# Tencent/hpc-ops

Hardware: AMD Instinct MI355X
Metric: attention_decode_fp8_kv_throughput (higher is better)
Workload: dtype fp8_e4m3

## Files before the change

### hpc-ops_amd/csrc/attention_decode_v2.h

```cpp
#pragma once
#include <hip/hip_runtime.h>
#include <stdint.h>

#include "attention_decode_route.h"

namespace hpc {
namespace decode2 {

struct Args {
  const void* q;
  const void* kcache;
  const void* vcache;
  const int* block_ids;
  const int* lens;
  const int* task_map;
  uint16_t* y;
  float* part_o;
  float* part_lse;
  int* arrive;
  const float* qscale;
  const float* kscale;
  const float* vscale;
  int num_batch, num_seq_q, num_head_kv, g_shift, page_shift, max_blocks;
  int ldq, ldy, qscale_stride, new_kv_included;
  int share_shift = 0;
  int min_range_cost;
  int bf16;
  int ktok = 0;
  int pair_wgs[4];
  int big_pct;
  int dev_nomem;
  int pair_xor;
  int mate_from;
  int xcd_map;
  int dev_sleep;
  int dev_merge_dup = 0;
  int dev_nosnap = 0;
  int dev_slice;
  long k_block_stride, k_token_stride;
  long v_block_stride, v_token_stride;
  long ks_block_stride, ks_row_stride, ks_head_stride;
  int hnd = 0;
  long k_head_stride = 0, v_head_stride = 0;
  float scale_log2;
  void* prof;
};

int launch(Args a, const DecodeRoute& r, hipStream_t stream);
#ifdef HPC_DEV
int ticket_overruns(bool reset);
#endif

}
}
```

### hpc-ops_amd/csrc/attention_decode_v2.hip

```cpp
#include <atomic>
#include <type_traits>
#include <utility>

#include "hpc_common.h"
#include "hpc_dev.h"
#include "../../include/hpc_amd.h"
#include "attention_decode_v2.h"

namespace hpc {
namespace decode2 {

#ifdef HPC_DEV
__device__ int g_ticket_overruns;
#endif
constexpr int kThreads = 256;
constexpr int kWaves = 4;
constexpr float kNegInf = -__builtin_inff();
constexpr int kRow = 256;
constexpr int kRows = 32;
constexpr int kVOff = kRows * kRow;
constexpr int kWaveLds = 2 * kRows * kRow;

template <int kAux>
__device__ __forceinline__ void ld_x4x4(u32x4 (&k)[4], int voff, i32x4 rs_in, int s1, int s2, int s3) {
  const i32x4 rs = pin(rs_in);
  if constexpr (kAux == 2)
    asm volatile("s_nop 4\n\tbuffer_load_dwordx4 %0, %4, %5, 0 offen nt\n\tbuffer_load_dwordx4 %1, %4, %5, %6 offen nt\n\t"
                 "buffer_load_dwordx4 %2, %4, %5, %7 offen nt\n\tbuffer_load_dwordx4 %3, %4, %5, %8 offen nt"
                 : "=&v"(k[0]), "=&v"(k[1]), "=&v"(k[2]), "=&v"(k[3])
                 : "v"(voff), "s"(rs), "s"(s1), "s"(s2), "s"(s3));
  else
    asm volatile("s_nop 4\n\tbuffer_load_dwordx4 %0, %4, %5, 0 offen\n\tbuffer_load_dwordx4 %1, %4, %5, %6 offen\n\t"
                 "buffer_load_dwordx4 %2, %4, %5, %7 offen\n\tbuffer_load_dwordx4 %3, %4, %5, %8 offen"
                 : "=&v"(k[0]), "=&v"(k[1]), "=&v"(k[2]), "=&v"(k[3])
                 : "v"(voff), "s"(rs), "s"(s1), "s"(s2), "s"(s3));
}
__device__ __forceinline__ void ld_q3(u32x4 (&q)[2], uint32_t& sc, int voff_q, i32x4 rq_in, int voff_s, i32x4 rsc_in) {
  const i32x4 rq = pin(rq_in), rsc = pin(rsc_in);
  asm volatile("s_nop 4\n\tbuffer_load_dwordx4 %0, %3, %4, 0 offen\n\tbuffer_load_dwordx4 %1, %3, %4, 0 offen offset:64\n\t"
               "buffer_load_dword %2, %5, %6, 0 offen"
               : "=&v"(q[0]), "=&v"(q[1]), "=&v"(sc)
               : "v"(voff_q), "s"(rq), "v"(voff_s), "s"(rsc));
}
__device__ __forceinline__ void ld_q4(u32x4 (&q)[4], int voff_q, i32x4 rq_in) {
  const i32x4 rq = pin(rq_in);
  asm volatile("s_nop 4\n\tbuffer_load_dwordx4 %0, %4, %5, 0 offen\n\tbuffer_load_dwordx4 %1, %4, %5, 0 offen offset:64\n\t"
               "buffer_load_dwordx4 %2, %4, %5, 0 offen offset:128\n\tbuffer_load_dwordx4 %3, %4, %5, 0 offen offset:192"
               : "=&v"(q[0]), "=&v"(q[1]), "=&v"(q[2]), "=&v"(q[3])
               : "v"(voff_q), "s"(rq));
}
__device__ __forceinline__ void ld_ks(uint32_t& sc, int voff, i32x4 rs_in) {
  const i32x4 rs = pin(rs_in);
  asm volatile("s_nop 4\n\tbuffer_load_dword %0, %1, %2, 0 offen" : "=&v"(sc) : "v"(voff), "s"(rs));
}
template <int N>
__device__ __forceinline__ void wait_ks(uint32_t& sc) {
  asm volatile("s_waitcnt vmcnt(%1)" : "+v"(sc) : "n"(N));
}
template <int N>
__device__ __forceinline__ void wait_ks2(uint32_t& sc0, uint32_t& sc1) {
  asm volatile("s_waitcnt vmcnt(%2)" : "+v"(sc0), "+v"(sc1) : "n"(N));
}
template <int N>
__device__ __forceinline__ void wait_q8(u32x4 (&q0)[4], u32x4 (&q1)[4]) {
  asm volatile("s_waitcnt vmcnt(%8)"
               : "+v"(q0[0]), "+v"(q0[1]), "+v"(q0[2]), "+v"(q0[3]), "+v"(q1[0]), "+v"(q1[1]), "+v"(q1[2]), "+v"(q1[3])
               : "n"(N < 63 ? N : 63));
}
template <int N>
__device__ __forceinline__ void wait_x4x4(u32x4 (&k)[4]) {
  asm volatile("s_waitcnt vmcnt(%4)" : "+v"(k[0]), "+v"(k[1]), "+v"(k[2]), "+v"(k[3]) : "n"(N < 63 ? N : 63));
}
template <int N>
__device__ __forceinline__ void wait_q(u32x4 (&q0)[2], u32x4 (&q1)[2], uint32_t& s0, uint32_t& s1) {
  asm volatile("s_waitcnt vmcnt(%6)" : "+v"(q0[0]), "+v"(q0[1]), "+v"(q1[0]), "+v"(q1[1]), "+v"(s0), "+v"(s1) : "n"(N < 63 ? N : 63));
}


constexpr int kFValid = 1;
constexpr int kFLast = 2;
constexpr int kFFirst = 4;
constexpr int kFOn0 = 8;
constexpr int kFOn1 = 16;
constexpr int kFMasked = 32;

template <int kAux, bool kBf16 = false, bool kProf = false, bool kQuad = false, bool kKtok = false, bool kHnd = false, bool kSolo = false>
__global__ __launch_bounds__(kThreads, 2) void decode2_kernel(const Args a) {
  static_assert(!kSolo || (!kQuad && !kHnd), "one head per workgroup: fp8 (both quant types) or bf16");
  static_assert(!(kSolo && kBf16 && kKtok), "bf16 has no scales");
  static_assert(!(kBf16 && kQuad), "the quad form is fp8");
  static_assert(!kKtok || (!kBf16 && !kQuad), "per-token K scales: the fp8 head-pair form");
  static_assert(!kHnd || (!kBf16 && !kQuad && !kKtok), "HND pages: the fp8 head-pair form with per-tensor scales");
  __shared__ float s_ks[kKtok ? kWaves : 1][64];
  constexpr bool kWide = (kBf16 && !kSolo) || kQuad;
  constexpr bool kBSolo = kBf16 && kSolo;
  __shared__ __attribute__((aligned(1024))) uint8_t s_wave[kWaves][kWaveLds];
  __shared__ float s_m[2][kWaves][16];
  __shared__ float s_l[2][kWaves][16];
  __shared__ int s_ticket[2];
  constexpr int kH = kSolo ? 1 : kQuad ? 4 : 2;
  constexpr int kW = kBSolo ? 32 : kSolo ? 64 : kWide ? 16 : 32;
  constexpr int kRowB = kBSolo ? 256 : kSolo ? 128 : kWide ? 512 : 256;
  constexpr int kRpi = kBSolo ? 4 : (kHnd || kSolo) ? 8 : kWide ? 2 : 4;
  constexpr int kCpr = 64 / kRpi;

  const int tid = threadIdx.x;
  const int lane = tid & 63;
  const int wave = sgpr(tid >> 6);
  const int n = lane & 15;
  const int g = lane >> 4;
  const int wg = blockIdx.x, nwg = gridDim.x;
  const int B = a.num_batch, Sq = a.num_seq_q;
  const int G = 1 << a.g_shift;
  const int rows_valid = Sq << a.g_shift;
  auto row_ok = [&](int r16, int hh = 0) __attribute__((always_inline)) { return (kQuad ? (r16 & 7) : kSolo ? 16 * hh + r16 : r16) < rows_valid; };
  const int page_mask = (1 << a.page_shift) - 1;
  const cint_ptr lens = as_const(a.lens);
  const int mpl_tiles = as_const(a.task_map)[6] >> 6;
  const int add_new = a.new_kv_included ? 0 : Sq;
  const uint8_t* qbase = static_cast<const uint8_t*>(a.q);
  const auto part_rs = make_rsrc(a.part_o);
  const auto lse_rs = make_rsrc(a.part_lse);
  auto ltot_of = [&](int b) __attribute__((always_inline)) { const int l = lens[b] + add_new; return l > 0 ? l : 0; };
  auto tiles_of = [&](int b) __attribute__((always_inline)) { return (ltot_of(b) + 63) >> 6; };

  constexpr int kOvh = 2;
  auto cost_of = [&](int b) __attribute__((always_inline)) { const int t = tiles_of(b); return t > 0 ? t + kOvh : 0; };
  const int kpl = (B + 63) >> 6;
  int chunk_sum = 0;
  for (int i = 0; i < kpl; ++i) {
    const int b = lane * kpl + i;
    if (b < B) {
      const int l = a.lens[b] + add_new;
      const int t = ((l > 0 ? l : 0) + 63) >> 6;
      chunk_sum += t > 0 ? t + kOvh : 0;
    }
  }
  int incl = chunk_sum;
  incl += __builtin_amdgcn_update_dpp(0, incl, 0x111, 0xF, 0xF, false);
  incl += __builtin_amdgcn_update_dpp(0, incl, 0x112, 0xF, 0xF, false);
  incl += __builtin_amdgcn_update_dpp(0, incl, 0x114, 0xF, 0xF, false);
  incl += __builtin_amdgcn_update_dpp(0, incl, 0x118, 0xF, 0xF, false);
  incl += __builtin_amdgcn_update_dpp(0, incl, 0x142, 0xA, 0xF, false);
  incl += __builtin_amdgcn_update_dpp(0, incl, 0x143, 0xC, 0xF, false);
  const int chunk_start = incl - chunk_sum;
  const int Th = __builtin_amdgcn_readlane(incl, 63);
  const int npair = a.num_head_kv / kH;
  if (Th == 0) return;
  int nrange = nwg / npair;
  int rng = wg / npair;
  int pr = wg % npair;
  if (a.xcd_map != 0 && npair == 4 && (nwg & 7) == 0) {
    const int e = (a.xcd_map >> (3 * (wg & 7))) & 7;
    pr = e & 3;
    rng = (wg >> 3) * 2 + (e >> 2);
  }
  if (a.mate_from > 0 && wg >= a.mate_from) pr ^= a.pair_xor;
  if constexpr (kSolo) {
    if (a.share_shift > 0) {
      const int ss = a.share_shift, hk = npair >> ss;
// ... 3 lines not shown
        rng = (j >> ss) * (8 / hk) + x / hk;
      } else {
        pr = ((pr % hk) << ss) | (pr / hk);
      }
    }
  }
  int lwg = wg;
  int lwg0 = pr * nrange;
  if (a.pair_wgs[0] > 0 && npair == 4) {
    const int n0 = a.pair_wgs[0], n1 = a.pair_wgs[1], n2 = a.pair_wgs[2], n3 = a.pair_wgs[3];
    const int nmin = min(min(n0, n1), min(n2, n3));
    if (wg >= nmin * 4) {
      int e = wg - nmin * 4;
      pr = 0;
      rng = nmin + e;
      if (e >= n0 - nmin) { e -= n0 - nmin; pr = 1; rng = nmin + e;
        if (e >= n1 - nmin) { e -= n1 - nmin; pr = 2; rng = nmin + e;
          if (e >= n2 - nmin) { e -= n2 - nmin; pr = 3; rng = nmin + e; } } }
    }
    nrange = pr == 0 ? n0 : pr == 1 ? n1 : pr == 2 ? n2 : n3;
    lwg0 = pr == 0 ? 0 : pr == 1 ? n0 : pr == 2 ? n0 + n1 : n0 + n1 + n2;
  }
  lwg = lwg0 + rng;
  const int nbig = a.big_pct > 100 ? (nwg / 2) / npair : 0;
  const long denom = static_cast<long>(nbig) * a.big_pct + static_cast<long>(nrange - nbig) * 100;
  const int per_s_even = static_cast<int>((static_cast<long>(Th) * 100 + denom - 1) / denom);
  const int per_floor = a.min_range_cost > mpl_tiles ? a.min_range_cost : mpl_tiles;
  const int per_s = per_s_even > per_floor ? per_s_even : per_floor;
  const int per_b = nbig > 0 ? (per_s * a.big_pct + 99) / 100 : per_s;
  const int big_span = nbig * per_b;
  auto range_of = [&](int pos) __attribute__((always_inline)) { return pos < big_span ? pos / per_b : nbig + (pos - big_span) / per_s; };
  const long g_begin = rng < nbig ? static_cast<long>(rng) * per_b : big_span + static_cast<long>(rng - nbig) * per_s;
  const int per = rng < nbig ? per_b : per_s;
  const long g_end = g_begin + per < Th ? g_begin + per : Th;
  if (g_begin >= g_end) return;

  constexpr int kSnap = 16;
  const bool snap = per_s_even <= per_floor && !(kHpcDevBuild && a.dev_nosnap);
  auto locate = [&](int x, int& b_out, int& rt_out, int& cc_out) __attribute__((always_inline)) {
    if (x >= Th) {
      b_out = B;
      rt_out = 0;
      cc_out = Th;
      return;
    }
    const uint64_t le = __ballot(chunk_start <= x);
    const int cl = 63 - __builtin_clzll(le);
    int pos = __builtin_amdgcn_readlane(chunk_start, cl);
    int b = cl * kpl;
    while (true) {
      const int t = cost_of(b);
      if (x < pos + t) break;
      pos += t;
      ++b;
    }
    if (snap && x > pos) {
      const int t = cost_of(b);
      if (t - kOvh <= kSnap) {
        if (2 * (x - pos) >= t) {
          pos += t;
          ++b;
          while (b < B && cost_of(b) == 0) ++b;
          if (b >= B) {
            b_out = B;
            rt_out = 0;
            cc_out = Th;
            return;
          }
        }
        b_out = b;
        rt_out = 0;
        cc_out = pos;
        return;
      }
    }
    b_out = b;
    rt_out = x - pos > kOvh ? x - pos - kOvh : 0;
    cc_out = pos;
  };
  int c_b, c_rt0, c_cc, e_b, e_rt, e_cc;
  locate(static_cast<int>(g_begin), c_b, c_rt0, c_cc);
  locate(static_cast<int>(g_end), e_b, e_rt, e_cc);
  if (c_b == e_b && c_rt0 >= e_rt) return;

  int q0_b = 0, q0_ltot = 0, q0_end = 0, q0_cc = 0;
  int q1_b = 0, q1_ltot = 0, q1_end = 0, q1_cc = 0;
  int q2_b = 0, q2_ltot = 0, q2_end = 0, q2_cc = 0;
  int qn = 0;
  int c_tok = 0, c_tok_end = 0, c_ltot = 0, c_tiles = 0, c_first = 1, c_valid = 1, c_pending = 0, c_last = 0;
  cint_ptr c_row = as_const(a.block_ids);
  auto open_task = [&]() __attribute__((always_inline)) {
    c_ltot = ltot_of(c_b);
    c_tiles = (c_ltot + 63) >> 6;
    const int end_t = c_b == e_b ? e_rt : c_tiles;
    c_tok_end = end_t * 64 < c_ltot ? end_t * 64 : c_ltot;
    c_tok = c_rt0 * 64 + wave * kW;
    c_first = 1;
    c_row = as_const(a.block_ids) + static_cast<long>(c_b) * a.max_blocks;
    const bool e0 = qn == 0, e1 = qn == 1, e2 = qn >= 2;
    q0_b = e0 ? c_b : q0_b, q0_ltot = e0 ? c_ltot : q0_ltot, q0_end = e0 ? c_tok_end : q0_end, q0_cc = e0 ? c_cc : q0_cc;
    q1_b = e1 ? c_b : q1_b, q1_ltot = e1 ? c_ltot : q1_ltot, q1_end = e1 ? c_tok_end : q1_end, q1_cc = e1 ? c_cc : q1_cc;
    q2_b = e2 ? c_b : q2_b, q2_ltot = e2 ? c_ltot : q2_ltot, q2_end = e2 ? c_tok_end : q2_end, q2_cc = e2 ? c_cc : q2_cc;
    ++qn;
  };
  auto next_task = [&]() __attribute__((always_inline)) {
    if (c_b == e_b) {
      c_valid = 0;
      return;
    }
    c_cc += c_tiles + kOvh;
    do {
      ++c_b;
    } while (c_b < e_b && tiles_of(c_b) == 0);
    if (c_b == e_b && e_rt == 0) {
      c_valid = 0;
      return;
    }
    c_rt0 = 0;
    open_task();
  };
  const bool blk1_same_page = (1 << a.page_shift) >= kW;
  auto step = [&](int& tok, int& fl, int& pid0, int& pid1) __attribute__((always_inline)) {
    if (c_pending && c_valid) {
      if (c_last) {
        next_task();
      } else {
        c_tok += kWaves * kW;
        c_first = 0;
      }
    }
    c_pending = 1;
    c_last = c_tok + kWaves * kW >= c_tok_end;
    const bool on0 = c_valid && c_tok < c_tok_end, on1 = c_valid && c_tok + kW / 2 < c_tok_end;
    const bool masked = c_tok + kW > c_ltot - Sq + 1 || c_tok + kW > c_tok_end;
    fl = (c_valid ? kFValid : 0) | (c_last ? kFLast : 0) | (c_first ? kFFirst : 0) | (on0 ? kFOn0 : 0) | (on1 ? kFOn1 : 0) |
         (masked ? kFMasked : 0);
    tok = c_tok;
    pid0 = on0 ? c_row[c_tok >> a.page_shift] : 0;
    pid1 = (!blk1_same_page && on1) ? c_row[(c_tok + kW / 2) >> a.page_shift] : 0;
  };

  u32x4 kr[2][4];
  u32x4 vr[2][4];
  uint32_t qsc[2];
  const uint32_t k_rs = static_cast<uint32_t>(a.k_token_stride), v_rs = static_cast<uint32_t>(a.v_token_stride);
  const int in0 = (wave * kW) & page_mask;
  const int in1 = blk1_same_page ? in0 + kW / 2 : ((wave * kW + kW / 2) & page_mask);
  const int lane_off = (lane % kCpr) * 16;
  const int k_voff0 = static_cast<int>((in0 + lane / kCpr) * k_rs) + lane_off, k_voff1 = static_cast<int>((in1 + lane / kCpr) * k_rs) + lane_off;
  const int v_voff0 = static_cast<int>((in0 + lane / kCpr) * v_rs) + lane_off, v_voff1 = static_cast<int>((in1 + lane / kCpr) * v_rs) + lane_off;
  const int ks1 = sgpr(kRpi * k_rs), ks2 = sgpr(kHnd ? static_cast<uint32_t>(a.k_head_stride) : 2 * kRpi * k_rs);
  const int ks3 = sgpr(kHnd ? static_cast<uint32_t>(a.k_head_stride) + kRpi * k_rs : 3 * kRpi * k_rs);
  const int vs1 = sgpr(kRpi * v_rs), vs2 = sgpr(kHnd ? static_cast<uint32_t>(a.v_head_stride) : 2 * kRpi * v_rs);
  const int vs3 = sgpr(kHnd ? static_cast<uint32_t>(a.v_head_stride) + kRpi * v_rs : 3 * kRpi * v_rs);
  const int mem_slice = kSolo ? (pr >> a.share_shift) : (a.dev_slice > 0 ? a.dev_slice - 1 : pr);
  const uint64_t kbase_h = reinterpret_cast<uint64_t>(a.kcache) + static_cast<uint64_t>(mem_slice) * (kSolo ? static_cast<uint64_t>(a.k_head_stride) : kHnd ? 2 * static_cast<uint64_t>(a.k_head_stride) : kRowB);
  const uint64_t vbase_h = reinterpret_cast<uint64_t>(a.vcache) + static_cast<uint64_t>(mem_slice) * (kSolo ? static_cast<uint64_t>(a.v_head_stride) : kHnd ? 2 * static_cast<uint64_t>(a.v_head_stride) : kRowB);
  const uint32_t kbs = static_cast<uint32_t>(a.k_block_stride), vbs = static_cast<uint32_t>(a.v_block_stride);
  const bool mem = a.dev_nomem == 0;
  i32x4 dk0, dk1, dv0, dv1;
  uint32_t ksr = 0;
  uint32_t ksr1 = 0;
  i32x4 dks = i32x4{0, 0, 0, kSrdWord3};
  i32x4 dks1 = i32x4{0, 0, 0, kSrdWord3};
  const uint64_t ksbase_h = reinterpret_cast<uint64_t>(a.kscale) + static_cast<uint64_t>(mem_slice) * (kSolo ? 1 : 2) * a.ks_head_stride +
                            static_cast<uint64_t>(in0 >> 5) * a.ks_row_stride;
  const uint64_t ksbase1_h = reinterpret_cast<uint64_t>(a.kscale) + static_cast<uint64_t>(mem_slice) * a.ks_head_stride +
                             static_cast<uint64_t>(blk1_same_page ? (in0 >> 5) + 1 : in1 >> 5) * a.ks_row_stride;
  const uint32_t ksbs = static_cast<uint32_t>(a.ks_block_stride);
  auto make_descs = [&](int fl, int pid0, int pid1) __attribute__((always_inline)) {
    const int nrec0 = (fl & kFOn0) && mem ? -1 : 0, nrec1 = (fl & kFOn1) && mem ? -1 : 0;
    const uint64_t ka = kbase_h + static_cast<uint64_t>(static_cast<uint32_t>(pid0)) * kbs;
    const uint64_t va = vbase_h + static_cast<uint64_t>(static_cast<uint32_t>(pid0)) * vbs;
    dk0 = srd(static_cast<uint32_t>(ka), static_cast<uint32_t>(ka >> 32), nrec0);
    dv0 = srd(static_cast<uint32_t>(va), static_cast<uint32_t>(va >> 32), nrec0);
    if (blk1_same_page) {
      dk1 = i32x4{dk0[0], dk0[1], sgpr(nrec1), kSrdWord3};
      dv1 = i32x4{dv0[0], dv0[1], sgpr(nrec1), kSrdWord3};
    } else {
      const uint64_t kb = kbase_h + static_cast<uint64_t>(static_cast<uint32_t>(pid1)) * kbs;
      const uint64_t vb = vbase_h + static_cast<uint64_t>(static_cast<uint32_t>(pid1)) * vbs;
      dk1 = srd(static_cast<uint32_t>(kb), static_cast<uint32_t>(kb >> 32), nrec1);
      dv1 = srd(static_cast<uint32_t>(vb), static_cast<uint32_t>(vb >> 32), nrec1);
    }
    if constexpr (kKtok) {
      const uint64_t sa = ksbase_h + static_cast<uint64_t>(static_cast<uint32_t>(pid0)) * ksbs;
      dks = srd(static_cast<uint32_t>(sa), static_cast<uint32_t>(sa >> 32), (fl & kFOn0) ? (kSolo ? 128 : 256) : 0);
      if constexpr (kSolo) {
        const uint64_t sb = ksbase1_h + static_cast<uint64_t>(static_cast<uint32_t>(blk1_same_page ? pid0 : pid1)) * ksbs;
        dks1 = srd(static_cast<uint32_t>(sb), static_cast<uint32_t>(sb >> 32), (fl & kFOn1) ? 128 : 0);
      }
    }
  };
  auto issue_k0 = [&]() __attribute__((always_inline)) { ld_x4x4<kAux>(kr[0], k_voff0, dk0, ks1, ks2, ks3); };
  auto issue_k1 = [&]() __attribute__((always_inline)) { ld_x4x4<kAux>(kr[1], k_voff1, dk1, ks1, ks2, ks3); };
  auto issue_v0 = [&]() __attribute__((always_inline)) { ld_x4x4<kAux>(vr[0], v_voff0, dv0, vs1, vs2, vs3); };
  auto issue_v1 = [&]() __attribute__((always_inline)) { ld_x4x4<kAux>(vr[1], v_voff1, dv1, vs1, vs2, vs3); };
// ... 61 lines not shown
      const i32x4 rq = srd_of(qbase + static_cast<long>(db) * Sq * a.ldq + ((pr * kH) << a.g_shift) * 128,
                              static_cast<unsigned>((Sq - 1) * a.ldq + kH * G * 128));
      const i32x4 rsq = srd_of(a.qscale + static_cast<long>(db) * Sq * a.qscale_stride + ((pr * kH) << a.g_shift),
                               static_cast<unsigned>(((Sq - 1) * a.qscale_stride + kH * G) * 4));
      ld_q3(reinterpret_cast<u32x4(&)[2]>(qf[0]), qsc[0], q_voff, rq, s_voff, rsq);
      ld_q3(reinterpret_cast<u32x4(&)[2]>(qf[1]), qsc[1], okc ? q_voff + 2 * G * 128 : -256, rq, okc ? s_voff + 2 * G * 4 : -256, rsq);
      return;
    }
    if constexpr (kSolo) {
      const i32x4 rq = srd_of(qbase + static_cast<long>(db) * Sq * a.ldq + (pr << a.g_shift) * 128,
                              static_cast<unsigned>((Sq - 1) * a.ldq + G * 128));
      const i32x4 rsq = srd_of(a.qscale + static_cast<long>(db) * Sq * a.qscale_stride + (pr << a.g_shift),
                               static_cast<unsigned>(((Sq - 1) * a.qscale_stride + G) * 4));
#pragma unroll
      for (int hh = 0; hh < 2; ++hh) {
        const int r = 16 * hh + n;
        ld_q3(reinterpret_cast<u32x4(&)[2]>(qf[hh]), qsc[hh], (r >> a.g_shift) * a.ldq + (r & (G - 1)) * 128 + g * 16, rq,
              ((r >> a.g_shift) * a.qscale_stride + (r & (G - 1))) * 4, rsq);
      }
      return;
    }
    const int q_voff = (n >> a.g_shift) * a.ldq + (n & (G - 1)) * 128 + g * 16;
    const int s_voff = ((n >> a.g_shift) * a.qscale_stride + (n & (G - 1))) * 4;
    const i32x4 rq = srd_of(qbase + static_cast<long>(db) * Sq * a.ldq + ((pr * kH) << a.g_shift) * 128,
                            static_cast<unsigned>((Sq - 1) * a.ldq + kH * G * 128));
    const i32x4 rsq = srd_of(a.qscale + static_cast<long>(db) * Sq * a.qscale_stride + ((pr * kH) << a.g_shift),
                             static_cast<unsigned>(((Sq - 1) * a.qscale_stride + kH * G) * 4));
    if constexpr (!kBf16) {
      ld_q3(reinterpret_cast<u32x4(&)[2]>(qf[0]), qsc[0], q_voff, rq, s_voff, rsq);
      ld_q3(reinterpret_cast<u32x4(&)[2]>(qf[1]), qsc[1], q_voff + G * 128, rq, s_voff + G * 4, rsq);
    }
  };
  auto reset_state = [&]() __attribute__((always_inline)) {
#pragma unroll
    for (int hh = 0; hh < 2; ++hh)
#pragma unroll
      for (int jj = 0; jj < 8; ++jj) o[hh][jj] = f32x4{0.f, 0.f, 0.f, 0.f};
#pragma unroll
    for (int hh = 0; hh < 2; ++hh) {
      m_run[hh] = kNegInf;
      l_run[hh] = 0.f;
    }
  };

  int p1_tok, p1_fl, p2_tok, p2_fl, p2_pid0, p2_pid1;

  auto combine4 = [&](int hh, int row16, int c8, float (&acc)[8], float& M, float& L) __attribute__((always_inline)) {
    float mw[kWaves];
    M = kNegInf;
#pragma unroll
    for (int w = 0; w < kWaves; ++w) {
      mw[w] = s_m[hh][w][row16];
      M = fmaxf(M, mw[w]);
    }
    const float Mu = M == kNegInf ? 0.f : M;
    L = 0.f;
#pragma unroll
    for (int i = 0; i < 8; ++i) acc[i] = 0.f;
#pragma unroll
    for (int w = 0; w < kWaves; ++w) {
      const float wgt = __builtin_amdgcn_exp2f(mw[w] - Mu);
      L += wgt * s_l[hh][w][row16];
      const float* so = reinterpret_cast<const float*>(s_wave[w]) + (hh * 16 + row16) * 128 + c8 * 8;
      const f32x4 x0 = *reinterpret_cast<const f32x4*>(so);
      const f32x4 x1 = *reinterpret_cast<const f32x4*>(so + 4);
#pragma unroll
      for (int i = 0; i < 4; ++i) {
        acc[i] = fmaf(wgt, x0[i], acc[i]);
        acc[4 + i] = fmaf(wgt, x1[i], acc[4 + i]);
      }
    }
  };
  auto store_y = [&](int db, int hh, int row16, int c8, const float (&acc)[8], float inv) __attribute__((always_inline)) {
    const int qrow = kQuad ? (row16 & 7) : kSolo ? 16 * hh + row16 : row16;
    const int rs = qrow >> a.g_shift;
    const int h = kQuad ? pr * kH + hh * 2 + (row16 >> 3) : kSolo ? pr : pr * kH + hh;
    uint16_t* dst = a.y + (static_cast<long>(db) * Sq + rs) * a.ldy + ((h << a.g_shift) + (qrow & (G - 1))) * 128 + c8 * 8;
    u32x4 pk;
#pragma unroll
    for (int i = 0; i < 4; ++i) pk[i] = pack_bf16x2(acc[2 * i] * inv, acc[2 * i + 1] * inv);
    st16(dst, pk);
  };

  int np = 0, p0_b = 0, p0_first = 0, p0_n = 0, p1_b = 0, p1_first = 0, p1_n = 0;
  auto merge_request = [&](int db, int first_rng, int nchunks) __attribute__((always_inline)) {
    int* cnt = a.arrive + static_cast<long>(pr) * B + db;
    const int r4 = lane >> 4, c8l = lane & 15;
    auto slot_of = [&](int c, int hh) __attribute__((always_inline)) {
      return (static_cast<long>(lwg0 + first_rng + c) * 2 + (c == 0 ? 1 : 0)) * 2 + hh;
    };
#pragma unroll 1
    for (int ig = 0; ig < 2; ++ig) {
      if (!kQuad && ig * 8 >= rows_valid) break;
      float um[2][2], ul[2][2], ua[2][2][8];
#pragma unroll
      for (int hh = 0; hh < 2; ++hh)
#pragma unroll
        for (int i = 0; i < 2; ++i) {
          um[hh][i] = kNegInf;
          ul[hh][i] = 0.f;
#pragma unroll
          for (int e = 0; e < 8; ++e) ua[hh][i][e] = 0.f;
        }
      for (int c0 = wave; c0 < nchunks; c0 += 2 * kWaves) {
        float lv[2][2][2];
        u32x4 x0[2][2][2], x1[2][2][2];
#pragma unroll
        for (int u = 0; u < 2; ++u) {
          const int c = c0 + u * kWaves < nchunks ? c0 + u * kWaves : c0;
          if (u > 0 && c0 + u * kWaves >= nchunks && !(kHpcDevBuild && a.dev_merge_dup)) continue;
#pragma unroll
          for (int hh = 0; hh < 2; ++hh) {
            const long slot = slot_of(c, hh);
#pragma unroll
            for (int i = 0; i < 2; ++i) {
              const int row = ig * 8 + i * 4 + r4;
              lv[u][hh][i] = __uint_as_float(__builtin_amdgcn_raw_buffer_load_b32(lse_rs, static_cast<int>((slot * 16 + row) * 4), 0, 16));
              const int off = static_cast<int>(((slot * 16 + row) * 128 + c8l * 8) * 4);
              x0[u][hh][i] = __builtin_amdgcn_raw_buffer_load_b128(part_rs, off, 0, 16);
              x1[u][hh][i] = __builtin_amdgcn_raw_buffer_load_b128(part_rs, off + 16, 0, 16);
            }
          }
        }
#pragma unroll
        for (int u = 0; u < 2; ++u) {
          const bool real = c0 + u * kWaves < nchunks;
          if (!real && !(kHpcDevBuild && a.dev_merge_dup)) continue;
#pragma unroll
          for (int hh = 0; hh < 2; ++hh)
#pragma unroll
            for (int i = 0; i < 2; ++i) {
              const float lse = real ? lv[u][hh][i] : kNegInf;
              const float mn = fmaxf(um[hh][i], lse);
              const float mu = mn == kNegInf ? 0.f : mn;
              const float sc_old = __builtin_amdgcn_exp2f(um[hh][i] - mu), wgt = __builtin_amdgcn_exp2f(lse - mu);
              um[hh][i] = mn;
              ul[hh][i] = ul[hh][i] * sc_old + wgt;
#pragma unroll
              for (int e = 0; e < 4; ++e) {
                ua[hh][i][e] = fmaf(wgt, __uint_as_float(x0[u][hh][i][e]), ua[hh][i][e] * sc_old);
                ua[hh][i][4 + e] = fmaf(wgt, __uint_as_float(x1[u][hh][i][e]), ua[hh][i][4 + e] * sc_old);
              }
            }
        }
      }
#pragma unroll
      for (int hh = 0; hh < 2; ++hh)
#pragma unroll
        for (int i = 0; i < 2; ++i) {
          const int row = ig * 8 + i * 4 + r4;
          if (c8l == 0) {
            s_m[hh][wave][row] = um[hh][i];
            s_l[hh][wave][row] = ul[hh][i];
          }
          float* so = my_so + (hh * 16 + row) * 128 + c8l * 8;
          *reinterpret_cast<f32x4*>(so) = f32x4{ua[hh][i][0], ua[hh][i][1], ua[hh][i][2], ua[hh][i][3]};
          *reinterpret_cast<f32x4*>(so + 4) = f32x4{ua[hh][i][4], ua[hh][i][5], ua[hh][i][6], ua[hh][i][7]};
        }
    }
    __syncthreads();
    const int row16 = tid >> 4, c8 = tid & 15;
#pragma unroll
    for (int hh = 0; hh < 2; ++hh) {
      if (row_ok(row16, hh)) {
        float acc[8], M, L;
        combine4(hh, row16, c8, acc, M, L);
        store_y(db, hh, row16, c8, acc, L > 0.f ? 1.0f / L : 0.f);
      }
    }
    if (tid == 0) __hip_atomic_store(cnt, 0, __ATOMIC_RELAXED, __HIP_MEMORY_SCOPE_AGENT);
    __syncthreads();
  };
  auto flush_pending = [&]() __attribute__((always_inline)) {
    if (np == 0) return;
    asm volatile("s_waitcnt vmcnt(0)" ::: "memory");
    __syncthreads();
    if (tid == 0) {
      s_ticket[0] = __hip_atomic_fetch_add(a.arrive + static_cast<long>(pr) * B + p0_b, 1, __ATOMIC_RELAXED, __HIP_MEMORY_SCOPE_AGENT) + 1;
      if (np > 1)
        s_ticket[1] = __hip_atomic_fetch_add(a.arrive + static_cast<long>(pr) * B + p1_b, 1, __ATOMIC_RELAXED, __HIP_MEMORY_SCOPE_AGENT) + 1;
    }
    __syncthreads();
    const int t0 = s_ticket[0], t1 = s_ticket[1];
#ifdef HPC_DEV
    if (tid == 0 && (t0 > p0_n || (np > 1 && t1 > p1_n))) atomicAdd(&g_ticket_overruns, 1);
#endif
    if (t0 == p0_n) merge_request(p0_b, p0_first, p0_n);
    if (np > 1 && t1 == p1_n) merge_request(p1_b, p1_first, p1_n);
    np = 0;
  };

  auto finish_task = [&]() __attribute__((always_inline)) {
    const int db = q0_b;
    const int d_tiles = (q0_ltot + 63) >> 6;
    const bool whole = snap && d_tiles <= kSnap;
    const int first_rng = whole ? rng : range_of(q0_cc + kOvh);
    const int nchunks = whole ? 1 : range_of(q0_cc + kOvh + d_tiles - 1) - first_rng + 1;
    const int ichunk = rng - first_rng;
#pragma unroll
    for (int hh = 0; hh < 2; ++hh) {
      const float l = row4_sum(l_run[hh]);
      if (g == 0) {
        s_m[hh][wave][n] = m_run[hh];
        s_l[hh][wave][n] = l;
      }
#pragma unroll
      for (int jj = 0; jj < 8; ++jj)
        *reinterpret_cast<f32x4*>(&my_so[(hh * 16 + n) * 128 + jj * 16 + g * 4]) = o[hh][jj];
    }
    __syncthreads();
    {
      const int row16 = tid >> 4, c8 = tid & 15;
#pragma unroll
      for (int hh = 0; hh < 2; ++hh) {
        float acc[8], M, L;
        combine4(hh, row16, c8, acc, M, L);
        const float inv = (L > 0.f ? 1.0f / L : 0.f) * (kKtok ? out_scale_h[hh] : out_scale);
        if (row_ok(row16, hh)) {
          if (nchunks == 1) {
            store_y(db, hh, row16, c8, acc, inv);
          } else {
            const long slot = (static_cast<long>(lwg) * 2 + (ichunk == 0 ? 1 : 0)) * 2 + hh;
            const int off = static_cast<int>(((slot * 16 + row16) * 128 + c8 * 8) * 4);
            __builtin_amdgcn_raw_buffer_store_b128(u32x4{__float_as_uint(acc[0] * inv), __float_as_uint(acc[1] * inv), __float_as_uint(acc[2] * inv),
                                                         __float_as_uint(acc[3] * inv)}, part_rs, off, 0, 16);
            __builtin_amdgcn_raw_buffer_store_b128(u32x4{__float_as_uint(acc[4] * inv), __float_as_uint(acc[5] * inv), __float_as_uint(acc[6] * inv),
                                                         __float_as_uint(acc[7] * inv)}, part_rs, off + 16, 0, 16);
            if (c8 == 0)
              __builtin_amdgcn_raw_buffer_store_b32(__float_as_uint(L > 0.f ? M + __builtin_amdgcn_logf(L) - (kBf16 ? 0.0f : 8.0f) : kNegInf),
                                                    lse_rs, static_cast<int>((slot * 16 + row16) * 4), 0, 16);
          }
        }
      }
    }
    if (nchunks > 1) {
      p1_b = np == 1 ? db : p1_b, p1_first = np == 1 ? first_rng : p1_first, p1_n = np == 1 ? nchunks : p1_n;
      p0_b = np == 0 ? db : p0_b, p0_first = np == 0 ? first_rng : p0_first, p0_n = np == 0 ? nchunks : p0_n;
      np = np < 2 ? np + 1 : 2;
    }
    __syncthreads();
    reset_state();
    q0_b = q1_b, q0_ltot = q1_ltot, q0_end = q1_end, q0_cc = q1_cc;
    q1_b = q2_b, q1_ltot = q2_ltot, q1_end = q2_end, q1_cc = q2_cc;
    --qn;
    if (p1_fl & kFValid) load_q(q0_b);
  };

  reset_state();
#pragma unroll
  for (int hh = 0; hh < 2; ++hh) {
#pragma unroll
    for (int c = 0; c < (kBf16 ? 4 : 2); ++c) qf[hh][c] = u32x4{0u, 0u, 0u, 0u};
    qsc[hh] = 0u;
  }
#pragma unroll
  for (int hh = 0; hh < 2; ++hh) row_scale[hh] = 0.f;
  out_scale = 0.f;
  open_task();
  step(p2_tok, p2_fl, p2_pid0, p2_pid1);
  make_descs(p2_fl, sgpr(p2_pid0), sgpr(p2_pid1));
  issue_k0();
  issue_k1();
  issue_ks();
  issue_v0();
  issue_v1();
  p1_tok = p2_tok;
  p1_fl = p2_fl;
  load_q(q0_b);
  step(p2_tok, p2_fl, p2_pid0, p2_pid1);

  uint64_t pf_wk = 0, pf_wr = 0, pf_wv = 0, pf_is = 0, pf_cp = 0, pf_fin = 0, pf_n = 0, pf_t0 = 0, pf_r0 = 0, pf_last = 0;
  auto now = [&]() __attribute__((always_inline)) -> uint64_t { return kProf ? __builtin_amdgcn_s_memtime() : 0; };
  if constexpr (kProf) {
    pf_t0 = now();
    pf_r0 = __builtin_amdgcn_s_memrealtime();
  }
  while (true) {
    const int d_tok = p1_tok, d_fl = p1_fl;
    if (!(d_fl & kFValid)) break;
    pf_last = now();
    uint32_t w0 = w0_inv, w1 = w1_inv, r0 = r0_inv, t0 = t0_inv;
    asm volatile("" : "+v"(w0), "+v"(w1), "+v"(r0), "+v"(t0));
    make_descs(p2_fl, sgpr(p2_pid0), sgpr(p2_pid1));
    p1_tok = p2_tok;
    p1_fl = p2_fl;
    auto write_k = [&](int tb) __attribute__((always_inline)) {
#pragma unroll
      for (int q = 0; q < 4; ++q) {
        if constexpr (kSolo && !kBf16)
          *reinterpret_cast<lds_u32x4*>(static_cast<uint32_t>((w0 ^ (((q >> 1) << 2) * 16)) + (tb * 32 + q * 8) * kRowB)) = kr[tb][q];
        else if constexpr (kHnd)
          *reinterpret_cast<lds_u32x4*>(static_cast<uint32_t>((w0 ^ ((((q >> 1) << 3) ^ ((q & 1) << 3) ^ (tb << 3)) * 16)) + (tb * 16 + (q & 1) * 8) * kRowB)) = kr[tb][q];
        else if constexpr (kWide)
          *reinterpret_cast<lds_u32x4*>(static_cast<uint32_t>((w0 ^ (((q << 1) ^ (tb << 3)) * 16)) + (tb * 8 + q * 2) * kRowB)) = kr[tb][q];
        else
          *reinterpret_cast<lds_u32x4*>(static_cast<uint32_t>((w0 ^ (((q << 2) ^ (tb << 3)) * 16)) + (tb * 16 + q * 4) * kRowB)) = kr[tb][q];
      }
    };
    auto write_v = [&](int tb) __attribute__((always_inline)) {
#pragma unroll
      for (int q = 0; q < 4; ++q) {
        if constexpr (kBSolo)
          *reinterpret_cast<lds_u32x4*>(static_cast<uint32_t>(w1 + (tb * 16 + q * 4) * kRowB)) = vr[tb][q];
        else if constexpr (kSolo)
          *reinterpret_cast<lds_u32x4*>(static_cast<uint32_t>((w0 ^ (((q >> 1) << 2) * 16)) + kVOff + (tb * 32 + q * 8) * kRowB)) = vr[tb][q];
        else if constexpr (kHnd)
          *reinterpret_cast<lds_u32x4*>(static_cast<uint32_t>((w0 ^ ((((q >> 1) << 3) ^ ((q & 1) << 3) ^ (tb << 3)) * 16)) + kVOff + (tb * 16 + (q & 1) * 8) * kRowB)) = vr[tb][q];
        else if constexpr (kBf16)
          *reinterpret_cast<lds_u32x4*>(static_cast<uint32_t>((w1 ^ (((q << 2) ^ tb) * 16)) + (tb * 8 + q * 2) * kRowB)) = vr[tb][q];
        else if constexpr (kQuad)
          *reinterpret_cast<lds_u32x4*>(static_cast<uint32_t>((w0 ^ (((q << 1) ^ (tb << 3)) * 16)) + kVOff + (tb * 8 + q * 2) * kRowB)) = vr[tb][q];
        else
          *reinterpret_cast<lds_u32x4*>(static_cast<uint32_t>((w0 ^ (((q << 2) ^ (tb << 3)) * 16)) + kVOff + (tb * 16 + q * 4) * kRowB)) = vr[tb][q];
      }
    };
    auto q_ready = [&]() __attribute__((always_inline)) {
      if (d_fl & kFFirst) {
        if constexpr (kBf16) {
          wait_q8<0>(qf[0], qf[1]);
          row_scale[0] = row_scale[1] = a.scale_log2;
          out_scale = 1.0f;
        } else {
          wait_q<0>(reinterpret_cast<u32x4(&)[2]>(qf[0]), reinterpret_cast<u32x4(&)[2]>(qf[1]), qsc[0], qsc[1]);
          const float kmul = kKtok ? 1.0f : as_constf(a.kscale)[0];
#pragma unroll
          for (int hh = 0; hh < 2; ++hh) row_scale[hh] = a.scale_log2 * __uint_as_float(qsc[hh]) * kmul;
          out_scale = as_constf(a.vscale)[0];
          if constexpr (kKtok) {
            out_scale_h[0] = as_constf(a.vscale)[kSolo ? (pr >> a.share_shift) : pr * 2];
            out_scale_h[1] = as_constf(a.vscale)[kSolo ? (pr >> a.share_shift) : pr * 2 + 1];
          }
        }
      }
    };
    constexpr int kNks = kKtok ? (kSolo ? 2 : 1) : 0;
    wait_x4x4<12 + kNks>(kr[0]);
    wait_x4x4<8 + kNks>(kr[1]);
    if constexpr (kProf) { const uint64_t t = now(); pf_wk += t - pf_last; pf_last = t; }
    write_k(0);
    write_k(1);
    if constexpr (kKtok && kSolo) {
      wait_ks2<8>(ksr, ksr1);
      s_ks[wave][lane] = __uint_as_float(lane < 32 ? ksr : ksr1);
    } else if constexpr (kKtok) {
      wait_ks<8>(ksr);
      s_ks[wave][lane] = __uint_as_float(ksr);
    }
    if constexpr (kProf) { const uint64_t t = now(); pf_wr += t - pf_last; pf_last = t; }
    wait_x4x4<4>(vr[0]);
    wait_x4x4<0>(vr[1]);
    if constexpr (kProf) { const uint64_t t = now(); pf_wv += t - pf_last; pf_last = t; }
    write_v(0);
    write_v(1);
    if constexpr (kProf) { const uint64_t t = now(); pf_wr += t - pf_last; pf_last = t; }
    if constexpr (kHpcDevBuild) {
      if (a.dev_sleep > 0 && !(pr & 1))
        for (int i = 0; i < a.dev_sleep; ++i) __builtin_amdgcn_s_sleep(1);
    }
    issue_k0();
    issue_k1();
    issue_ks();
    issue_v0();
    issue_v1();
    q_ready();
    step(p2_tok, p2_fl, p2_pid0, p2_pid1);
    if constexpr (kProf) { const uint64_t t = now(); pf_is += t - pf_last; pf_last = t; }

    if constexpr (kBSolo) {
      f32x4 sacc[2][2];
#pragma unroll
      for (int tb = 0; tb < 2; ++tb) {
        f32x4 acc[2] = {f32x4{0.f, 0.f, 0.f, 0.f}, f32x4{0.f, 0.f, 0.f, 0.f}};
#pragma unroll
        for (int j = 0; j < 4; ++j) {
          const u32x4 kk = *reinterpret_cast<const lds_u32x4*>(static_cast<uint32_t>((r0 ^ (((j << 2) ^ (tb << 3)) * 16)) + tb * 16 * kRowB));
#pragma unroll
          for (int hh = 0; hh < 2; ++hh)
            acc[hh] = __builtin_amdgcn_mfma_f32_16x16x32_bf16(__builtin_bit_cast(bf16x8, kk), __builtin_bit_cast(bf16x8, qf[hh][j]), acc[hh], 0, 0, 0);
        }
        sacc[0][tb] = acc[0];
        sacc[1][tb] = acc[1];
      }
      v4i16 pf[2][2];
#pragma unroll
      for (int hh = 0; hh < 2; ++hh)
#pragma unroll
        for (int tb = 0; tb < 2; ++tb)
#pragma unroll
          for (int r = 0; r < 4; ++r) sacc[hh][tb][r] *= row_scale[hh];
      if (d_fl & kFMasked) {
#pragma unroll
        for (int hh = 0; hh < 2; ++hh) {
          const int sq_row = (16 * hh + n) >> a.g_shift;
          const int lim = (q0_end - 1 < q0_ltot - Sq + sq_row) ? q0_end - 1 : q0_ltot - Sq + sq_row;
#pragma unroll
          for (int tb = 0; tb < 2; ++tb)
#pragma unroll
            for (int r = 0; r < 4; ++r) sacc[hh][tb][r] = (d_tok + tb * 16 + g * 4 + r) <= lim ? sacc[hh][tb][r] : kNegInf;
        }
      }
#pragma unroll
      for (int hh = 0; hh < 2; ++hh) {
        float mt = kNegInf;
#pragma unroll
        for (int tb = 0; tb < 2; ++tb)
#pragma unroll
          for (int r = 0; r < 4; ++r) mt = __builtin_fmaxf(mt, sacc[hh][tb][r]);
        mt = row4_max(mt);
        const float m_new = fmaxf(m_run[hh], mt);
        const float m_use = m_new == kNegInf ? 0.f : m_new;
        float psum = 0.f;
#pragma unroll
        for (int tb = 0; tb < 2; ++tb) {
          float prb[4];
#pragma unroll
          for (int r = 0; r < 4; ++r) {
            prb[r] = __builtin_amdgcn_exp2f(sacc[hh][tb][r] - m_use);
            psum += prb[r];
// ... 314 lines not shown
            prb[r] = __builtin_amdgcn_exp2f(sacc[hh][tb][r] - m8);
            psum += prb[r];
          }
          int w = __builtin_amdgcn_cvt_pk_fp8_f32(prb[0], prb[1], 0, false);
          w = __builtin_amdgcn_cvt_pk_fp8_f32(prb[2], prb[3], w, true);
          pf[hh][tb] = static_cast<uint32_t>(w);
        }
        if (__builtin_amdgcn_ballot_w64(m_new != m_run[hh]) != 0) {
          const float alpha = __builtin_amdgcn_exp2f(m_run[hh] - m_use);
          l_run[hh] *= alpha;
  #pragma unroll
          for (int jj = 0; jj < 8; ++jj) o[hh][jj] *= alpha;
          m_run[hh] = m_new;
        }
        l_run[hh] += psum;
      }

      constexpr int kTrBatch = 8;
  #pragma unroll
      for (int hh = 0; hh < 2; ++hh)
  #pragma unroll
        for (int j4 = 0; j4 < 8; j4 += kTrBatch) {
          v2i32 vt[kTrBatch];
  #pragma unroll
          for (int u = 0; u < kTrBatch; ++u)
            vt[u] = __builtin_amdgcn_ds_read_tr8_b64_v2i32(
                reinterpret_cast<lds_v2i32*>(static_cast<uint32_t>(t0 ^ (((hh << 3) | (j4 + u)) * 16))));
          __builtin_amdgcn_sched_barrier(0);
  #pragma unroll
          for (int u = 0; u < kTrBatch; ++u)
            o[hh][j4 + u] = __builtin_amdgcn_mfma_f32_16x16x32_fp8_fp8(
                pack64(static_cast<uint32_t>(vt[u][0]), static_cast<uint32_t>(vt[u][1])), pack64(pf[hh][0], pf[hh][1]),
                o[hh][j4 + u], 0, 0, 0);
          __builtin_amdgcn_sched_barrier(0);
        }
    }
    if constexpr (kProf) {
      asm volatile("s_nop 0" ::"v"(o[0][0]), "v"(o[1][7]));
      const uint64_t t = now();
      pf_cp += t - pf_last;
      pf_last = t;
      ++pf_n;
    }
    if (d_fl & kFLast) {
      finish_task();
      if constexpr (kProf) { const uint64_t t = now(); pf_fin += t - pf_last; pf_last = t; }
    }
  }
  if constexpr (kProf) {
    if (lane == 0 && a.prof) {
      const uint64_t t1 = now(), r1 = __builtin_amdgcn_s_memrealtime();
      uint64_t* dst = reinterpret_cast<uint64_t*>(a.prof) + (static_cast<long>(wg) * kWaves + wave) * 12;
      dst[0] = pf_r0, dst[1] = r1, dst[2] = t1 - pf_t0, dst[3] = pf_wk, dst[4] = pf_wv, dst[5] = pf_wr, dst[6] = pf_is, dst[7] = pf_cp,
      dst[8] = pf_fin, dst[9] = pf_n, dst[10] = __builtin_amdgcn_s_getreg((4 << 0) | (0 << 6) | (31 << 11)) ,
      dst[11] = (static_cast<uint64_t>(__builtin_amdgcn_s_getreg((20 << 0) | (0 << 6) | (31 << 11)) ) << 32) |
                (static_cast<uint64_t>(rng) << 8) | static_cast<uint64_t>(pr);
    }
  }
  flush_pending();
  asm volatile("s_waitcnt vmcnt(0)" ::: "memory");
}

#ifdef HPC_DEV
int ticket_overruns(bool reset) {
  int v = 0;
  if (hipMemcpyFromSymbol(&v, HIP_SYMBOL(g_ticket_overruns), sizeof(int)) != hipSuccess) return -1;
  const int zero = 0;
  if (reset && hipMemcpyToSymbol(HIP_SYMBOL(g_ticket_overruns), &zero, sizeof(int)) != hipSuccess) return -1;
  return v;
}
#endif

static void set_grid_params(Args& a, const DecodeRoute& r) {
  int dev = 0;
  const int cus = hipGetDevice(&dev) == hipSuccess ? hpc_get_cu_count(dev) : 0;
  const int num_wg = r.num_wg;
  const bool pairs = r.mode != 3;
  const int units = pairs ? a.num_head_kv / (r.mode == 2 ? 4 : 2) : a.num_head_kv;
  a.dev_slice = pairs ? hpc_dev_tuning_get(kDevDecodeOneSlice) : 0;
  a.xcd_map = pairs ? hpc_dev_tuning_get(kDevDecodeXcdMap) : 0;
  a.dev_sleep = pairs ? hpc_dev_tuning_get(kDevDecodeSleep) : 0;
  a.dev_merge_dup = pairs && hpc_dev_tuning_get(kDevDecodeMergeDup) == 1;
  a.dev_nosnap = pairs && hpc_dev_tuning_get(kDevDecodeNoSnap) == 1;
  {
    const int k36 = hpc_dev_tuning_get(kDevDecodePairSwizzle);
    const int mask = k36 > 0 ? k36 - 1 : !pairs ? 0 : (a.bf16 || r.mode == 2 || units == 2) ? 1 : 2;
    const bool ok = cus > 0 && num_wg > cus && (units & (units - 1)) == 0 && mask > 0 && mask < units && cus % units == 0 &&
                    (!a.hnd || k36 > 0);
    a.pair_xor = ok ? mask : 0;
    a.mate_from = ok ? cus : 0;
  }
  a.pair_wgs[0] = a.pair_wgs[1] = a.pair_wgs[2] = a.pair_wgs[3] = 0;
  if (!a.bf16 && r.mode == 1 && a.num_head_kv == 8 && num_wg >= 256 && num_wg % 4 == 0) {
    const int k30 = hpc_dev_tuning_get(kDevDecodeExtraWg256), k31 = hpc_dev_tuning_get(kDevDecodeExtraWg768);
    const int even = num_wg / 4;
    int d1 = (k30 != 0 ? k30 - 100 : 0) * even / 128, d3 = (k31 != 0 ? k31 - 100 : 0) * even / 128;
    if (d1 != 0 || d3 != 0) {
      const int give = d1 + d3, g0 = give / 2, g2 = give - g0;
      a.pair_wgs[0] = even - g0, a.pair_wgs[1] = even + d1, a.pair_wgs[2] = even - g2, a.pair_wgs[3] = even + d3;
    }
  }
  if (a.pair_wgs[0] > 0) a.pair_xor = a.mate_from = 0;
  const int k32 = hpc_dev_tuning_get(kDevDecodeFirstHalfPct);
  a.big_pct = pairs && k32 > 100 && k32 <= 200 && cus > 0 && num_wg == 2 * cus && (num_wg / 2) % units == 0 ? k32 : 100;
}

int launch(Args a, const DecodeRoute& r, hipStream_t stream) {
  set_grid_params(a, r);
  const bool temporal = hpc_dev_tuning_get(kDevDecodeKvTemporal) == 1, solo = r.mode == 3, quad = r.mode == 2;
#define HPC_DECODE2(...) decode2_kernel<__VA_ARGS__><<<r.num_wg, kThreads, 0, stream>>>(a)
  if (solo && a.bf16)                           HPC_DECODE2(2, true,  false, false, false, false, true);
  else if (solo && a.ktok)                      HPC_DECODE2(2, false, false, false, true,  false, true);
  else if (kHpcDevBuild && solo && a.prof)      HPC_DECODE2(2, false, true,  false, false, false, true);
  else if (solo)                                HPC_DECODE2(2, false, false, false, false, false, true);
  else if (a.ktok)                              HPC_DECODE2(2, false, false, false, true);
  else if (kHpcDevBuild && a.hnd && a.prof)     HPC_DECODE2(2, false, true,  false, false, true);
  else if (a.hnd)                               HPC_DECODE2(2, false, false, false, false, true);
  else if (temporal && a.bf16)                  HPC_DECODE2(0, true);
  else if (a.bf16)                              HPC_DECODE2(2, true);
  else if (kHpcDevBuild && quad && a.prof)      HPC_DECODE2(2, false, true,  true);
  else if (kHpcDevBuild && temporal && quad)    HPC_DECODE2(0, false, false, true);
  else if (kHpcDevBuild && quad)                HPC_DECODE2(2, false, false, true);
  else if (kHpcDevBuild && a.prof)              HPC_DECODE2(2, false, true);
  else if (temporal)                            HPC_DECODE2(0);
  else                                          HPC_DECODE2(2);
#undef HPC_DECODE2
  if (hipGetLastError() == hipSuccess) return HPC_OK;
  (void)hipMemsetAsync(a.arrive, 0, kCounterBytes, stream);
  (void)hipGetLastError();
  return HPC_ERR_LAUNCH;
}

}
}
```

### hpc-ops_amd/csrc/hpc_dev.h

```cpp
#pragma once

enum DevKey : int {
  kDevDecodeKvTemporal = 0,
  kDevStreamGemmForm = 1,
  kDevGgemmTiledMode = 3,
  kDevDecodeNoWaveSolo = 5,
  kDevTiled256Form = 6,
  kDevPrefillRowMap = 7,
  kDevArRuntimeWorld = 9,
  kDevArSpinLog2 = 10,
  kDevArMinGrid = 11,
  kDevDecodeFp8NoPair = 12,
  kDevDecodeGrid = 14,
  kDevDecodeNoKvLoads = 15,
  kDevP8NoDma = 18,
  kDevMoeSplitAct = 19,
  kDevDecodeMinRangeCost = 20,
  kDevP8NoHalfTile = 21,
  kDevP8LoopVariant = 22,
  kDevP8TailsLast = 23,
  kDevP8TailTemporal = 24,
  kDevGgemmP8From192 = 25,
  kDevP8TailRegs = 26,
  kDevDecodeBf16NoPair = 28,
  kDevDecodeQuadForm = 29,
  kDevDecodeExtraWg256 = 30,
  kDevDecodeExtraWg768 = 31,
  kDevDecodeFirstHalfPct = 32,
  kDevDecodeCombineKernel = 33,
  kDevSchedBins = 34,
  kDevArLlLaunches = 35,
  kDevDecodePairSwizzle = 36,
  kDevDecodeOneSlice = 37,
  kDevDecodeXcdMap = 38,
  kDevDecodeSleep = 39,
  kDevRouterGemm64 = 40,
  kDevRouterGemmSkipLoads = 41,
  kDevP8ItemScanOld = 43,
  kDevRouterGemmSplitCap = 45,
  kDevPrefillBf16Perm = 46,
  kDevArCasBarrier = 47,
  kDevArPackedFlags = 48,
  kDevP8NoRideAlong = 49,
  kDevArLlOneShot = 52,
  kDevArLlNoNorm = 53,
  kDevDecodeQt0FirstGen = 54,
  kDevDecodeHndPair = 55,
  kDevStreamGemmLoop = 56,
  kDevDecodeMergeDup = 58,
  kDevDecodeSoloForm = 60,
  kDevDecodeNoSnap = 61,
};

#ifdef HPC_DEV
constexpr bool kHpcDevBuild = true;
extern "C" int hpc_dev_tuning_set(int key, int value);
extern "C" int hpc_dev_tuning_get(int key);
#else
constexpr bool kHpcDevBuild = false;
static constexpr int hpc_dev_tuning_get(int) { return 0; }
#endif
```

Baseline: 5756.

## Reorder split-task processing, issue merge tickets early, relax Q wait count

Workgroups whose range spans several batches now process the trailing partial chunk first and return to the leading partial chunk last, so the split-KV pieces that need merging finish earlier. The arrival-counter atomic for each pending merge is issued asynchronously right after partial results are written to LDS, and its result is collected later in flush_pending. This overlaps the atomic's latency with the output stores. The first-tile Q wait now lets the younger K loads stay in flight instead of draining all of vmcnt. Dev-only flags can restore the old behaviours. The costs are more scheduling state and inline-asm atomics whose correctness depends on the vmcnt ordering.

```diff
diff --git a/hpc-ops_amd/csrc/attention_decode_v2.h b/hpc-ops_amd/csrc/attention_decode_v2.h
--- a/hpc-ops_amd/csrc/attention_decode_v2.h
+++ b/hpc-ops_amd/csrc/attention_decode_v2.h
@@ -36,6 +36,7 @@
   int dev_sleep;
   int dev_merge_dup = 0;
   int dev_nosnap = 0;
+  int dev_task_ends = 0;
   int dev_slice;
   long k_block_stride, k_token_stride;
   long v_block_stride, v_token_stride;
diff --git a/hpc-ops_amd/csrc/attention_decode_v2.hip b/hpc-ops_amd/csrc/attention_decode_v2.hip
--- a/hpc-ops_amd/csrc/attention_decode_v2.hip
+++ b/hpc-ops_amd/csrc/attention_decode_v2.hip
@@ -75,7 +75,13 @@
 __device__ __forceinline__ void wait_q(u32x4 (&q0)[2], u32x4 (&q1)[2], uint32_t& s0, uint32_t& s1) {
   asm volatile("s_waitcnt vmcnt(%6)" : "+v"(q0[0]), "+v"(q0[1]), "+v"(q1[0]), "+v"(q1[1]), "+v"(s0), "+v"(s1) : "n"(N < 63 ? N : 63));
 }
-
+__device__ __forceinline__ void take_ticket(uint32_t& t, const int* base, int byte_off) {
+  asm volatile("s_nop 4\n\tglobal_atomic_add %0, %1, %2, %3 sc0" : "+v"(t) : "v"(byte_off), "v"(1), "s"(base) : "memory");
+}
+template <int N>
+__device__ __forceinline__ void ticket_landed(uint32_t& t) {
+  asm volatile("s_waitcnt vmcnt(%1)" : "+v"(t) : "n"(N) : "memory");
+}
 
 constexpr int kFValid = 1;
 constexpr int kFLast = 2;
@@ -245,6 +251,11 @@
   locate(static_cast<int>(g_begin), c_b, c_rt0, c_cc);
   locate(static_cast<int>(g_end), e_b, e_rt, e_cc);
   if (c_b == e_b && c_rt0 >= e_rt) return;
+  const bool dev_q_drain = kHpcDevBuild && (a.dev_task_ends & 1), dev_in_order = kHpcDevBuild && (a.dev_task_ends & 2),
+             dev_late_tickets = kHpcDevBuild && (a.dev_task_ends & 4);
+  const bool chunk_first = c_b != e_b && e_rt > 0 && !dev_in_order;
+  const int w_b = c_b;
+  int c_order = 0;
 
   int q0_b = 0, q0_ltot = 0, q0_end = 0, q0_cc = 0;
   int q1_b = 0, q1_ltot = 0, q1_end = 0, q1_cc = 0;
@@ -267,6 +278,12 @@
     ++qn;
   };
   auto next_task = [&]() __attribute__((always_inline)) {
+    if (c_order == 1) {
+      c_order = 2;
+      c_b = w_b, c_rt0 = e_rt, c_cc = e_cc;
+      open_task();
+      return;
+    }
     if (c_b == e_b) {
       c_valid = 0;
       return;
@@ -275,7 +292,7 @@
     do {
       ++c_b;
     } while (c_b < e_b && tiles_of(c_b) == 0);
-    if (c_b == e_b && e_rt == 0) {
+    if (c_b == e_b && (c_order == 2 || e_rt == 0)) {
       c_valid = 0;
       return;
     }
@@ -503,7 +520,8 @@
     st16(dst, pk);
   };
 
-  int np = 0, p0_b = 0, p0_first = 0, p0_n = 0, p1_b = 0, p1_first = 0, p1_n = 0;
+  int np = 0, p0_b = 0, p0_first = 0, p0_n = 0, p1_b = 0, p1_first = 0, p1_n = 0, nt = 0;
+  uint32_t tk = 0;
   auto merge_request = [&](int db, int first_rng, int nchunks) __attribute__((always_inline)) {
     int* cnt = a.arrive + static_cast<long>(pr) * B + db;
     const int r4 = lane >> 4, c8l = lane & 15;
@@ -595,11 +613,18 @@
   auto flush_pending = [&]() __attribute__((always_inline)) {
     if (np == 0) return;
     asm volatile("s_waitcnt vmcnt(0)" ::: "memory");
-    __syncthreads();
-    if (tid == 0) {
-      s_ticket[0] = __hip_atomic_fetch_add(a.arrive + static_cast<long>(pr) * B + p0_b, 1, __ATOMIC_RELAXED, __HIP_MEMORY_SCOPE_AGENT) + 1;
-      if (np > 1)
-        s_ticket[1] = __hip_atomic_fetch_add(a.arrive + static_cast<long>(pr) * B + p1_b, 1, __ATOMIC_RELAXED, __HIP_MEMORY_SCOPE_AGENT) + 1;
+    if (nt < np) {
+      __syncthreads();
+      if (tid == 0) {
+        if (nt == 0)
+          s_ticket[0] = __hip_atomic_fetch_add(a.arrive + static_cast<long>(pr) * B + p0_b, 1, __ATOMIC_RELAXED, __HIP_MEMORY_SCOPE_AGENT) + 1;
+        if (np > 1)
+          s_ticket[1] = __hip_atomic_fetch_add(a.arrive + static_cast<long>(pr) * B + p1_b, 1, __ATOMIC_RELAXED, __HIP_MEMORY_SCOPE_AGENT) + 1;
+      }
+    }
+    if (tid < nt) {
+      ticket_landed<0>(tk);
+      s_ticket[tid] = static_cast<int>(tk) + 1;
     }
     __syncthreads();
     const int t0 = s_ticket[0], t1 = s_ticket[1];
@@ -608,7 +633,7 @@
 #endif
     if (t0 == p0_n) merge_request(p0_b, p0_first, p0_n);
     if (np > 1 && t1 == p1_n) merge_request(p1_b, p1_first, p1_n);
-    np = 0;
+    np = nt = 0;
   };
 
   auto finish_task = [&]() __attribute__((always_inline)) {
@@ -630,6 +655,10 @@
         *reinterpret_cast<f32x4*>(&my_so[(hh * 16 + n) * 128 + jj * 16 + g * 4]) = o[hh][jj];
     }
     __syncthreads();
+    if (nt < np && !dev_late_tickets) {
+      if (tid == nt) take_ticket(tk, a.arrive, static_cast<int>((static_cast<long>(pr) * B + (nt == 0 ? p0_b : p1_b)) * 4));
+      ++nt;
+    }
     {
       const int row16 = tid >> 4, c8 = tid & 15;
 #pragma unroll
@@ -677,7 +706,14 @@
 #pragma unroll
   for (int hh = 0; hh < 2; ++hh) row_scale[hh] = 0.f;
   out_scale = 0.f;
-  open_task();
+  if (chunk_first) {
+    const int rt0 = c_rt0, cc = c_cc;
+    c_b = e_b, c_rt0 = 0, c_cc = e_cc;
+    open_task();
+    e_rt = rt0, e_cc = cc, c_order = 1;
+  } else {
+    open_task();
+  }
   step(p2_tok, p2_fl, p2_pid0, p2_pid1);
   make_descs(p2_fl, sgpr(p2_pid0), sgpr(p2_pid1));
   issue_k0();
@@ -735,14 +771,18 @@
           *reinterpret_cast<lds_u32x4*>(static_cast<uint32_t>((w0 ^ (((q << 2) ^ (tb << 3)) * 16)) + kVOff + (tb * 16 + q * 4) * kRowB)) = vr[tb][q];
       }
     };
+    constexpr int kNks = kKtok ? (kSolo ? 2 : 1) : 0;
     auto q_ready = [&]() __attribute__((always_inline)) {
+      constexpr int kYounger = 16 + kNks;
       if (d_fl & kFFirst) {
         if constexpr (kBf16) {
-          wait_q8<0>(qf[0], qf[1]);
+          if (dev_q_drain) wait_q8<0>(qf[0], qf[1]);
+          else wait_q8<kYounger>(qf[0], qf[1]);
           row_scale[0] = row_scale[1] = a.scale_log2;
           out_scale = 1.0f;
         } else {
-          wait_q<0>(reinterpret_cast<u32x4(&)[2]>(qf[0]), reinterpret_cast<u32x4(&)[2]>(qf[1]), qsc[0], qsc[1]);
+          if (dev_q_drain) wait_q<0>(reinterpret_cast<u32x4(&)[2]>(qf[0]), reinterpret_cast<u32x4(&)[2]>(qf[1]), qsc[0], qsc[1]);
+          else wait_q<kYounger>(reinterpret_cast<u32x4(&)[2]>(qf[0]), reinterpret_cast<u32x4(&)[2]>(qf[1]), qsc[0], qsc[1]);
           const float kmul = kKtok ? 1.0f : as_constf(a.kscale)[0];
 #pragma unroll
           for (int hh = 0; hh < 2; ++hh) row_scale[hh] = a.scale_log2 * __uint_as_float(qsc[hh]) * kmul;
@@ -754,7 +794,6 @@
         }
       }
     };
-    constexpr int kNks = kKtok ? (kSolo ? 2 : 1) : 0;
     wait_x4x4<12 + kNks>(kr[0]);
     wait_x4x4<8 + kNks>(kr[1]);
     if constexpr (kProf) { const uint64_t t = now(); pf_wk += t - pf_last; pf_last = t; }
@@ -1235,6 +1274,7 @@
   a.dev_sleep = pairs ? hpc_dev_tuning_get(kDevDecodeSleep) : 0;
   a.dev_merge_dup = pairs && hpc_dev_tuning_get(kDevDecodeMergeDup) == 1;
   a.dev_nosnap = pairs && hpc_dev_tuning_get(kDevDecodeNoSnap) == 1;
+  a.dev_task_ends = hpc_dev_tuning_get(kDevDecodeTaskEnds);
   {
     const int k36 = hpc_dev_tuning_get(kDevDecodePairSwizzle);
     const int mask = k36 > 0 ? k36 - 1 : !pairs ? 0 : (a.bf16 || r.mode == 2 || units == 2) ? 1 : 2;
diff --git a/hpc-ops_amd/csrc/hpc_dev.h b/hpc-ops_amd/csrc/hpc_dev.h
--- a/hpc-ops_amd/csrc/hpc_dev.h
+++ b/hpc-ops_amd/csrc/hpc_dev.h
@@ -50,6 +50,7 @@
   kDevDecodeMergeDup = 58,
   kDevDecodeSoloForm = 60,
   kDevDecodeNoSnap = 61,
+  kDevDecodeTaskEnds = 62,
 };
 
 #ifdef HPC_DEV
```

Result: no change. 5726 (-0.5%).
